# risc0/zeth

Measured on AMD Instinct MI355X. Metric: segments/sec, higher is better.
Workload: dtype u32

## Files before the change

### zeth_amd/csrc/common.h

```cpp
#pragma once
#include <hip/hip_runtime.h>

#include <atomic>
#include <cstdarg>
#include <cstdio>
#include <cstdlib>
#include <cstring>
#include <map>
#include <string>
#include <vector>

#include "../../include/zkhal.h"
#include "fp.h"
#include "noise.h"

namespace zkh {

inline const char* make_err(const char* fmt, ...) {
    char buf[512];
    va_list ap;
    va_start(ap, fmt);
    vsnprintf(buf, sizeof buf, fmt, ap);
    va_end(ap);
    return strdup(buf);
}
#define ZKH_HIP(expr)                                                                               \
    do {                                                                                            \
        hipError_t _e = (expr);                                                                     \
        if (_e != hipSuccess) return zkh::make_err("%s failed: %s (%s:%d)", #expr, hipGetErrorString(_e), __FILE__, __LINE__); \
    } while (0)
#define ZKH_TRY(expr)                    \
    do {                                 \
        const char* _err = (expr);       \
        if (_err) return _err;           \
    } while (0)
#define ZKH_REQUIRE(cond, ...)                         \
    do {                                               \
        if (!(cond)) return zkh::make_err(__VA_ARGS__); \
    } while (0)

constexpr int ZKH_P2_PTAB = 486;
constexpr int TW_BITS = 12;
constexpr int TW_SIZE = 1 << TW_BITS;
constexpr int TW_HI_BITS = 14;
constexpr int TW_HI_SIZE = 1 << TW_HI_BITS;
constexpr int MAX_LOG_N = TW_BITS + TW_HI_BITS;
constexpr int LDS_TW_LOG = 12;

struct DeviceTables {
    uint32_t* rc;
    uint32_t* diag;
    uint32_t* tw_fwd_lo; uint32_t* tw_fwd_hi;
    uint32_t* tw_rev_lo; uint32_t* tw_rev_hi;
    uint32_t* tile_fwd;  uint32_t* tile_rev;
    uint32_t* layer_fwd; uint32_t* layer_rev;
    uint32_t* layer_fwd_lazy;
    uint32_t* shift_lo;  uint32_t* shift_hi;
};

struct ProfAgg { uint64_t calls = 0; double ms = 0; double bytes = 0; };
struct ProfPending { std::string name; hipEvent_t a, b; double bytes; };

}

struct zkh_alloc_t {
    void* ptr;
    size_t bytes;
    std::atomic<int> refs;
    bool owned;
    zkh_ctx* ctx;
    zkh_alloc_t(void* p, size_t b, int r, bool o, zkh_ctx* c) : ptr(p), bytes(b), refs(r), owned(o), ctx(c) {}
};

struct zkh_buf {
    zkh_alloc_t* a;
    size_t off, len;
    std::atomic<int> refs;
    zkh_buf(zkh_alloc_t* al, size_t o, size_t l, int r) : a(al), off(o), len(l), refs(r) {}
    uint32_t* ptr() const { return (uint32_t*)a->ptr + off; }
};

struct zkh_ctx {
    int device;
    hipStream_t stream;
    zkh::DeviceTables tab;
    uint32_t rou_fwd[28], rou_rev[28];
    uint32_t h_rc[24 * 29], h_diag[zkh::ZKH_P2_PTAB];
    std::multimap<size_t, void*> pool;
    size_t pool_bytes = 0, live_bytes = 0, peak_bytes = 0;
    bool prof = false;
    std::vector<zkh::ProfPending> pending;
    std::map<std::string, zkh::ProfAgg> agg;
    std::vector<hipEvent_t> event_pool;
    uint32_t* pinned = nullptr;
    size_t pinned_words = 0;
    size_t stage_next = 0, stage_used = 0;
    uint32_t* d_fail = nullptr;
    uint32_t* h_fail = nullptr;
    bool fail_armed = false;
    std::map<void*, size_t> host_blocks;
    size_t h2d_bytes = 0;
};

namespace zkh {

const char* pool_alloc(zkh_ctx* c, size_t bytes, void** out);
void pool_free(zkh_ctx* c, void* p, size_t bytes);
const char* new_buf(zkh_ctx* c, size_t n_words, bool zero, zkh_buf** out);
void prof_begin(zkh_ctx* c, const char* name, double bytes);
void prof_end(zkh_ctx* c);
const char* ensure_pinned(zkh_ctx* c, size_t words);
const char* resolve_noise_key(const uint32_t* key_or_null, NoiseKey* out);

inline void bind_thread(const zkh_ctx* c) { (void)hipSetDevice(c->device); }
const char* ntt_device_init(zkh_ctx* c);

struct Tmp {
    zkh_buf* b = nullptr;
    Tmp() {}
    Tmp(const Tmp&) = delete;
    Tmp& operator=(const Tmp&) = delete;
    ~Tmp() { if (b) zkh_release(b); }
    zkh_buf** out() { if (b) { zkh_release(b); b = nullptr; } return &b; }
    operator zkh_buf*() const { return b; }
    zkh_buf* operator->() const { return b; }
    explicit operator bool() const { return b != nullptr; }
};

struct ProfScope {
    zkh_ctx* c;
    ProfScope(zkh_ctx* ctx, const char* name, double bytes) : c(ctx) { bind_thread(c); if (c->prof) prof_begin(c, name, bytes); }
    ~ProfScope() { if (c->prof) prof_end(c); }
};

inline const char* last_launch_error(const char* what) {
    hipError_t e = hipGetLastError();
    if (e != hipSuccess) return make_err("launch %s: %s", what, hipGetErrorString(e));
    return nullptr;
}

__device__ __forceinline__ uint32_t xcd_remap(uint32_t b, uint32_t nblocks) {
    const uint32_t xcd = b & 7u, q = nblocks >> 3, r = nblocks & 7u, idx = b >> 3;
    const uint32_t base = xcd < r ? xcd * (q + 1) : r * (q + 1) + (xcd - r) * q;
    return base + idx;
}

}
```

### zeth_amd/csrc/hash.hip

```cpp
#include "common.h"
#include "image_tree.h"
#include "poseidon2.h"
#include "poseidon2_wide.h"

using namespace zkh;

static_assert(zkh::ZKH_P2_PTAB == zkh::P2_TAB_WORDS, "common.h ZKH_P2_PTAB must equal poseidon2.h P2_TAB_WORDS");

namespace {

__global__ __launch_bounds__(256, 4) void k_hash_rows(uint32_t* __restrict__ out, const uint32_t* __restrict__ matrix,
                                                   size_t rows, uint32_t cols, const uint32_t* __restrict__ rc,
                                                   const uint32_t* __restrict__ diag) {
    const size_t r = (size_t)blockIdx.x * blockDim.x + threadIdx.x;
    if (r >= rows) return;
    uint32_t s[CELLS];
#pragma unroll
    for (int i = 0; i < CELLS; i++) s[i] = 0;
    const uint32_t* src = matrix + r;
    const uint32_t full = cols / RATE, tail = cols % RATE;
    const uint32_t blocks = full + (tail || cols == 0 ? 1u : 0u);
    for (uint32_t b = 0; b < blocks; b++) {
        const uint32_t* bsrc = src + (size_t)b * RATE * rows;
        if (b < full) {
#pragma unroll
            for (int i = 0; i < RATE; i++) s[i] = bsrc[(size_t)i * rows];
        } else {
#pragma unroll
            for (int i = 0; i < RATE; i++) s[i] = (uint32_t)i < tail ? bsrc[(size_t)i * rows] : 0u;
        }
        poseidon2_mix_sponge(s, rc, diag, b + 1 == blocks);
#pragma unroll
        for (int i = RATE; i < CELLS; i++) s[i] = p2_signed(s[i]);
    }
#pragma unroll
    for (int i = 0; i < OUT; i++) s[i] = canon((int32_t)s[RATE + i]);
    uint4* o = (uint4*)(out + r * 8);
    o[0] = make_uint4(s[0], s[1], s[2], s[3]);
    o[1] = make_uint4(s[4], s[5], s[6], s[7]);
}

__device__ __forceinline__ void fold_one(uint32_t* __restrict__ io, size_t input_size, size_t output_size, size_t i,
                                         const uint32_t* __restrict__ rc, const uint32_t* __restrict__ diag) {
    const uint4* src = (const uint4*)(io + (input_size + 2 * i) * 8);
    uint32_t s[CELLS];
    const uint4 a = src[0], b = src[1], c = src[2], d = src[3];
    s[0] = a.x; s[1] = a.y; s[2] = a.z; s[3] = a.w; s[4] = b.x; s[5] = b.y; s[6] = b.z; s[7] = b.w;
    s[8] = c.x; s[9] = c.y; s[10] = c.z; s[11] = c.w; s[12] = d.x; s[13] = d.y; s[14] = d.z; s[15] = d.w;
#pragma unroll
    for (int k = RATE; k < CELLS; k++) s[k] = 0;
    poseidon2_mix_raw<0, OUT, RATE>(s, rc, diag);
#pragma unroll
    for (int k = 0; k < OUT; k++) s[k] = p2_finish(s[k]);
    uint4* o = (uint4*)(io + (output_size + i) * 8);
    o[0] = make_uint4(s[0], s[1], s[2], s[3]);
    o[1] = make_uint4(s[4], s[5], s[6], s[7]);
}
__global__ __launch_bounds__(256, 4) void k_hash_fold(uint32_t* __restrict__ io, size_t input_size, size_t output_size,
                                                   const uint32_t* __restrict__ rc, const uint32_t* __restrict__ diag) {
    const size_t i = (size_t)blockIdx.x * blockDim.x + threadIdx.x;
    if (i >= output_size) return;
    fold_one(io, input_size, output_size, i, rc, diag);
}
__global__ __launch_bounds__(256, 4) void k_hash_fold_list(uint32_t* __restrict__ io, size_t width, const uint32_t* __restrict__ list,
                                                        const uint32_t* __restrict__ count, const uint32_t* __restrict__ rc,
                                                        const uint32_t* __restrict__ diag) {
    const uint32_t t = blockIdx.x * blockDim.x + threadIdx.x;
    if (t >= *count) return;
    fold_one(io, 2 * width, width, list[t], rc, diag);
}

__device__ __forceinline__ void wide_fold_one(uint32_t* __restrict__ io, size_t input_size, size_t output_size, uint32_t gid,
                                              const uint32_t* rcs, const uint32_t* __restrict__ pc) {
    const uint32_t j = gid & 7;
    size_t parent = gid >> 3;
    const bool live = parent < output_size;
    if (!live) parent = output_size - 1;
    uint32_t c[4] = {0, 0, 0, 0};
    if (j < 4) {
        const uint4 v = *(const uint4*)(io + (input_size + 2 * parent) * 8 + 4 * j);
        c[0] = v.x; c[1] = v.y; c[2] = v.z; c[3] = v.w;
    }
    wide_permute(c, j, rcs, pc);
    if (live && j < 2) *(uint4*)(io + (output_size + parent) * 8 + 4 * j) = make_uint4(c[0], c[1], c[2], c[3]);
}
constexpr int TAIL_LOG = 7;
__global__ __launch_bounds__(8 << TAIL_LOG) void k_hash_fold_subtree(uint32_t* __restrict__ io, size_t first_parents, uint32_t levels,
                                                                     const uint32_t* __restrict__ rc, const uint32_t* __restrict__ pc) {
    __shared__ __attribute__((aligned(16))) uint32_t rcs[ROUNDS_TOTAL * CELLS + 8];
    for (uint32_t w = threadIdx.x; w < ROUNDS_TOTAL * CELLS; w += blockDim.x) rcs[w] = rc[w];
    __syncthreads();
    for (uint32_t l = 0; l < levels; l++) {
        const size_t parents = first_parents >> l;
        const uint32_t local = (1u << TAIL_LOG) >> l;
        if ((threadIdx.x >> 6) * 8 < local) {
            const uint32_t grp = threadIdx.x >> 3;
            const uint32_t gid = grp < local ? (uint32_t)((blockIdx.x * local + grp) * 8 + (threadIdx.x & 7)) : 0xffffffffu;
            wide_fold_one(io, 2 * parents, parents, gid, rcs, pc);
        }
        __threadfence_block();
        __syncthreads();
    }
}
__global__ __launch_bounds__(8 << TAIL_LOG) void k_hash_fold_tail(uint32_t* __restrict__ io, size_t first_parents,
                                                                  const uint32_t* __restrict__ rc, const uint32_t* __restrict__ pc) {
    __shared__ __attribute__((aligned(16))) uint32_t rcs[ROUNDS_TOTAL * CELLS + 8];
    for (uint32_t w = threadIdx.x; w < ROUNDS_TOTAL * CELLS; w += blockDim.x) rcs[w] = rc[w];
    __syncthreads();
    for (size_t parents = first_parents; parents >= 1; parents >>= 1) {
        if ((threadIdx.x >> 6) * 8 < parents)
            wide_fold_one(io, 2 * parents, parents, threadIdx.x, rcs, pc);
        __threadfence_block();
        __syncthreads();
    }
}

__global__ __launch_bounds__(256) void k_poseidon2_mix(uint32_t* __restrict__ io, size_t count, const uint32_t* __restrict__ rc,
                                                       const uint32_t* __restrict__ diag) {
    const size_t i = (size_t)blockIdx.x * blockDim.x + threadIdx.x;
    if (i >= count) return;
    uint4* p = (uint4*)(io + i * CELLS);
    uint32_t s[CELLS];
#pragma unroll
    for (int q = 0; q < CELLS / 4; q++) { const uint4 v = p[q]; s[4 * q] = v.x; s[4 * q + 1] = v.y; s[4 * q + 2] = v.z; s[4 * q + 3] = v.w; }
    poseidon2_mix(s, rc, diag);
#pragma unroll
    for (int q = 0; q < CELLS / 4; q++) p[q] = make_uint4(s[4 * q], s[4 * q + 1], s[4 * q + 2], s[4 * q + 3]);
}

}

extern "C" const char* zkh_poseidon2_mix(zkh_ctx* c, zkh_buf* states, size_t count) {
    ZKH_REQUIRE(states && states->len == count * CELLS, "poseidon2_mix: buffer is not count x 24 words");
    if (!count) return nullptr;
    bind_thread(c);
    k_poseidon2_mix<<<(unsigned)((count + 255) / 256), 256, 0, c->stream>>>(states->ptr(), count, c->tab.rc, c->tab.diag);
    return last_launch_error("poseidon2_mix");
}
extern "C" const char* zkh_hash_rows(zkh_ctx* c, zkh_buf* out, const zkh_buf* matrix) {
    ZKH_REQUIRE(out->len % 8 == 0 && out->len, "hash_rows: output is not a digest array");
    const size_t rows = out->len / 8;
    ZKH_REQUIRE(matrix->len % rows == 0, "hash_rows: matrix size %zu not a multiple of rows %zu", matrix->len, rows);
    const size_t cols = matrix->len / rows;
    ProfScope prof(c, "hash_rows", 4.0 * matrix->len + 32.0 * rows);
    k_hash_rows<<<(unsigned)((rows + 255) / 256), 256, 0, c->stream>>>(out->ptr(), matrix->ptr(), rows, (uint32_t)cols,
                                                                      c->tab.rc, c->tab.diag);
    return last_launch_error("hash_rows");
}
extern "C" const char* zkh_hash_fold(zkh_ctx* c, zkh_buf* io, size_t input_size, size_t output_size) {
    ZKH_REQUIRE(io->len % 8 == 0, "hash_fold: not a digest array");
    ZKH_REQUIRE((input_size + 2 * output_size) * 8 <= io->len && output_size * 2 <= input_size, "hash_fold: ranges out of bounds");
    if (!output_size) return nullptr;
    ProfScope prof(c, "hash_fold", 96.0 * output_size);
    k_hash_fold<<<(unsigned)((output_size + 255) / 256), 256, 0, c->stream>>>(io->ptr(), input_size, output_size, c->tab.rc,
                                                                             c->tab.diag);
    return last_launch_error("hash_fold");
}
extern "C" const char* zkh_merkle_fold_all(zkh_ctx* c, zkh_buf* nodes, size_t rows) {
    ZKH_REQUIRE(nodes->len == rows * 16 && rows && (rows & (rows - 1)) == 0, "merkle_fold_all: nodes must hold 2*rows digests");
    return merkle_fold_from(c, nodes, rows);
}
extern "C" const char* zkh_merkle_build(zkh_ctx* c, zkh_buf* nodes, const zkh_buf* matrix, size_t rows) {
    ZKH_REQUIRE(nodes && matrix && nodes->len == rows * 16 && rows && (rows & (rows - 1)) == 0, "merkle_build: nodes must hold 2*rows digests");
    ZKH_REQUIRE(matrix->len % rows == 0, "merkle_build: matrix size %zu not a multiple of rows %zu", matrix->len, rows);
    zkh_buf* leaves = nullptr;
    ZKH_TRY(zkh_slice(nodes, rows * 8, rows * 8, &leaves));
    const char* err = zkh_hash_rows(c, leaves, matrix);
    zkh_release(leaves);
    ZKH_TRY(err);
    return merkle_fold_from(c, nodes, rows);
}
const char* zkh::merkle_fold_from(zkh_ctx* c, zkh_buf* nodes, size_t first_layer) {
    for (size_t layer = first_layer; layer >= 2; layer /= 2) {
        const size_t parents = layer / 2;
        if (parents > ((size_t)1 << WIDE_LOG)) {
            ZKH_TRY(zkh_hash_fold(c, nodes, layer, parents));
        } else if (parents > ((size_t)1 << TAIL_LOG)) {
            uint32_t levels = 0;
            while ((parents >> levels) > ((size_t)1 << TAIL_LOG)) levels++;
            ProfScope prof(c, "hash_fold_wide", 96.0 * (2 * parents - (parents >> (levels - 1))));
            k_hash_fold_subtree<<<(unsigned)(parents >> TAIL_LOG), 8 << TAIL_LOG, 0, c->stream>>>(nodes->ptr(), parents, levels, c->tab.rc,
                                                                                                   c->tab.diag);
            ZKH_TRY(last_launch_error("hash_fold_wide"));
            layer >>= (levels - 1);
        } else {
            ProfScope prof(c, "hash_fold_tail", 96.0 * (2 * parents - 1));
            k_hash_fold_tail<<<1, 8 << TAIL_LOG, 0, c->stream>>>(nodes->ptr(), parents, c->tab.rc, c->tab.diag);
            ZKH_TRY(last_launch_error("hash_fold_tail"));
            break;
        }
    }
    return nullptr;
}
const char* zkh::hash_fold_listed(zkh_ctx* c, zkh_buf* nodes, size_t width, const uint32_t* list, const uint32_t* count, uint32_t bound) {
    ZKH_REQUIRE(bound && bound <= width && 32 * width <= nodes->len, "hash_fold_listed: %u parents of %zu in %zu words", bound, width, nodes->len);
    ProfScope prof(c, "image_sparse", 100.0 * bound);
    k_hash_fold_list<<<(bound + 255) / 256, 256, 0, c->stream>>>(nodes->ptr(), width, list, count, c->tab.rc, c->tab.diag);
    return last_launch_error("image_sparse");
}
```

### zeth_amd/csrc/poseidon2.h

```cpp
#pragma once
#include "fp.h"

namespace zkh {

constexpr int CELLS = 24, RATE = 16, OUT = 8, HALF_FULL = 4, PARTIAL = 21, ROUNDS_TOTAL = 2 * HALF_FULL + PARTIAL;
constexpr int P2_TAB_SIGNED = 74, P2_TAB_FULL = P2_TAB_SIGNED + 3 * CELLS, P2_TAB_GROUP0 = P2_TAB_FULL + 2 * HALF_FULL * CELLS,
              P2_TAB_KAPPA = P2_TAB_GROUP0 + 3 * CELLS, P2_TAB_EXIT = P2_TAB_KAPPA + 4, P2_TAB_WORDS = P2_TAB_EXIT + 3 * CELLS;

ZKH_HD uint32_t sbox7_rc(uint32_t x, uint32_t rcs) {
    const int32_t sx = (int32_t)(x + rcs);
    const int32_t x2 = smont(sx, sx), x3 = smont(x2, sx), x4 = smont(x2, x2);
    return canon(smont(x3, x4));
}
ZKH_HD uint32_t dbl_mod(uint32_t x) {
#if defined(__HIP_DEVICE_COMPILE__)
    uint32_t d;
    asm("v_add_u32_e32 %0, %1, %1" : "=v"(d) : "v"(x));
    return reduce_once(d);
#else
    return reduce_once(x + x);
#endif
}
ZKH_HD void m4(uint32_t& x0, uint32_t& x1, uint32_t& x2, uint32_t& x3) {
    const uint32_t t0 = add_mod(x0, x1), t1 = add_mod(x2, x3);
    const uint32_t t2 = add_mod(dbl_mod(x1), t1), t3 = add_mod(dbl_mod(x3), t0);
    const uint32_t t4 = add_mod(dbl_mod(dbl_mod(t1)), t3), t5 = add_mod(dbl_mod(dbl_mod(t0)), t2);
    x0 = add_mod(t3, t5); x1 = t5; x2 = add_mod(t2, t4); x3 = t4;
}
ZKH_HD void m_ext(uint32_t (&s)[CELLS]) {
    uint32_t c0 = 0, c1 = 0, c2 = 0, c3 = 0;
#pragma unroll
    for (int i = 0; i < CELLS; i += 4) {
        m4(s[i], s[i + 1], s[i + 2], s[i + 3]);
        c0 = add_mod(c0, s[i]); c1 = add_mod(c1, s[i + 1]); c2 = add_mod(c2, s[i + 2]); c3 = add_mod(c3, s[i + 3]);
    }
#pragma unroll
    for (int i = 0; i < CELLS; i += 4) {
        s[i] = add_mod(s[i], c0); s[i + 1] = add_mod(s[i + 1], c1);
        s[i + 2] = add_mod(s[i + 2], c2); s[i + 3] = add_mod(s[i + 3], c3);
    }
}
constexpr uint32_t F64_OFF = 0x43380000u;
constexpr double F64_MAGIC = 6755399441055744.0;

ZKH_HD int64_t f64_bits(double d) {
#if defined(__HIP_DEVICE_COMPILE__)
    return __double_as_longlong(d);
#else
    int64_t b; __builtin_memcpy(&b, &d, 8); return b;
#endif
}
ZKH_HD double fmad(double a, double b, double c) {
#if defined(__HIP_DEVICE_COMPILE__)
    return __builtin_fma(a, b, c);
#else
    return a * b + c;
#endif
}
ZKH_HD void m4d(double& x0, double& x1, double& x2, double& x3) {
    const double t0 = x0 + x1, t1 = x2 + x3;
    const double t2 = fmad(x1, 2.0, t1), t3 = fmad(x3, 2.0, t0);
    const double t4 = fmad(t1, 4.0, t3), t5 = fmad(t0, 4.0, t2);
    x0 = t3 + t5; x1 = t5; x2 = t2 + t4; x3 = t4;
}
ZKH_HD uint32_t m_ext_f64_cell(double tm) {
    const int64_t t = f64_bits(tm);
    const int32_t m = (int32_t)((uint32_t)t * NEG_PINV);
    return (uint32_t)((uint64_t)mad_i64_k(m, (int32_t)P, t) >> 32);
}
template <int LIVE>
ZKH_HD void m_ext_f64_blocks(double (&d)[CELLS], double (&c)[4]) {
    static_assert(LIVE % 4 == 0 && LIVE > 0 && LIVE <= CELLS, "whole 4-cell blocks");
    c[0] = c[1] = c[2] = c[3] = F64_MAGIC;
#pragma unroll
    for (int i = 0; i < LIVE; i += 4) {
        m4d(d[i], d[i + 1], d[i + 2], d[i + 3]);
        c[0] += d[i]; c[1] += d[i + 1]; c[2] += d[i + 2]; c[3] += d[i + 3];
    }
}
template <int LIVE, int SRC_LO, int DST_LO, int N>
ZKH_HD void m_ext_f64_reduce(uint32_t (&s)[CELLS], const double (&d)[CELLS], const double (&c)[4]) {
    static_assert(SRC_LO % 4 == 0 && DST_LO % 4 == 0 && SRC_LO + N <= CELLS && DST_LO + N <= CELLS, "column-aligned cell range");
#pragma unroll
    for (int k = 0; k < N; k++) s[DST_LO + k] = m_ext_f64_cell(SRC_LO + k < LIVE ? d[SRC_LO + k] + c[k % 4] : c[k % 4]);
}
ZKH_HD void m_ext_f64(uint32_t (&s)[CELLS], double (&d)[CELLS]) {
    double c[4];
    m_ext_f64_blocks<CELLS>(d, c);
    m_ext_f64_reduce<CELLS, 0, 0, CELLS>(s, d, c);
}
ZKH_HD uint64_t fold64(uint64_t a, uint64_t t) {
#if defined(__HIP_DEVICE_COMPILE__)
    uint64_t d, carry;
    asm("v_mad_u64_u32 %0, %1, %2, %3, %4" : "=v"(d), "=s"(carry) : "v"((uint32_t)(a >> 32)), "s"(R1), "v"(t));
    asm("v_mad_u64_u32 %0, %1, %2, 1, %3" : "=v"(t), "=s"(carry) : "v"((uint32_t)a), "v"(d));
    return t;
#else
    return t + (a >> 32) * R1 + (uint32_t)a;
#endif
}
ZKH_HD int32_t sbox7_lazy(uint32_t v, uint32_t rcf) {
    const int32_t sx = (int32_t)(v + rcf);
    const int32_t x2 = smont(sx, sx), x3 = smont(x2, sx), x4 = smont(x2, x2);
    return smont(x3, x4);
}

inline uint32_t p2_mulm(uint32_t a, uint32_t b) { return (uint32_t)((uint64_t)a * b % P); }
inline uint32_t p2_powm(uint32_t a, uint64_t e) { uint32_t r = 1; while (e) { if (e & 1) r = p2_mulm(r, a); a = p2_mulm(a, a); e >>= 1; } return r; }
inline uint32_t p2_full_round_scale(uint32_t lambda) { return p2_mulm(p2_powm(lambda, 7), p2_powm(p2_powm(R1, P - 2), 7)); }
inline uint32_t p2_exit_scale() {
    uint64_t e = 0;
    for (uint64_t k = 1; k < 7 && !e; k++) if ((k * (P - 1) + 1) % 7 == 0) e = (k * (P - 1) + 1) / 7;
    uint32_t lambda = R1;
    for (int f = 0; f < HALF_FULL; f++) lambda = p2_mulm(p2_powm(lambda, e), R1);
    return lambda;
}
inline bool poseidon2_partial_table(uint32_t* t, const uint32_t* rc_canonical, const uint32_t* diag_canonical) {
    Fp c1 = Fp::zero();
    for (int i = 0; i < CELLS; i++) {
        const Fp d = fp_encode(diag_canonical[i]);
        t[i] = d.v; t[CELLS + i] = (d * d).v; t[2 * CELLS + i] = (d * d * d).v;
        if (i) c1 = c1 + d;
    }
    t[3 * CELLS] = c1.v; t[3 * CELLS + 1] = fp_encode(23).v;
    for (int i = 0; i < 3 * CELLS; i++) t[P2_TAB_SIGNED + i] = (uint32_t)center(t[i]);
    const uint32_t rinv = p2_powm(R1, P - 2);
    auto rneg = [&](uint64_t k) { return p2_powm(rinv, k); };
    const uint32_t sigma = p2_exit_scale();
    uint32_t lam[2 * HALF_FULL + 1] = {1u, rneg(7), rneg(56), rneg(399), sigma};
    for (int f = HALF_FULL; f < 2 * HALF_FULL; f++) lam[f + 1] = p2_full_round_scale(lam[f]);
    for (int f = 0; f < 2 * HALF_FULL; f++) {
        const int round = f < HALF_FULL ? f : HALF_FULL + PARTIAL + (f - HALF_FULL);
        for (int i = 0; i < CELLS; i++) {
            const uint32_t v = p2_mulm(lam[f], rc_canonical[round * CELLS + i] % P);
            t[P2_TAB_FULL + f * CELLS + i] = f == HALF_FULL ? v - P : (uint32_t)center(v) - F64_OFF;
        }
    }
    const uint32_t rho = p2_powm(R1, 2801);
    for (int i = 0; i < 3 * CELLS; i++) t[P2_TAB_GROUP0 + i] = (uint32_t)center(p2_mulm(t[i], rho));
    t[P2_TAB_KAPPA] = (uint32_t)center(p2_mulm(rho, R1));
    t[P2_TAB_KAPPA + 1] = p2_mulm(rho, R1);
    const uint32_t mu = p2_mulm(sigma, rinv);
    t[P2_TAB_KAPPA + 2] = sigma;
    t[P2_TAB_KAPPA + 3] = p2_mulm(t[0], mu);
    for (int i = 0; i < 3 * CELLS; i++) t[P2_TAB_EXIT + i] = (uint32_t)center(p2_mulm(t[i], mu));
    return lam[2 * HALF_FULL] == R1;
}
ZKH_HD uint32_t p2_signed(uint32_t v) { return v - F64_OFF; }
ZKH_HD uint32_t p2_finish(uint32_t v) { return canon((int32_t)p2_signed(v)); }
template <int KEEP_LO, int KEEP_N, int LIVE, bool SEL>
ZKH_HD void poseidon2_mix_core(uint32_t (&s)[CELLS], const uint32_t* __restrict__ rc, const uint32_t* __restrict__ diag, bool low) {
    static_assert(!SEL || KEEP_LO >= KEEP_N, "the two selectable ranges do not overlap");
    const uint32_t* __restrict__ rcf = diag + P2_TAB_FULL;
    double d[CELLS], c[4];
#pragma unroll
    for (int i = 0; i < LIVE; i++) d[i] = (double)(int32_t)s[i];
    m_ext_f64_blocks<LIVE>(d, c);
    m_ext_f64_reduce<LIVE, 0, 0, CELLS>(s, d, c);
#pragma unroll 1
    for (int r = 0; r < HALF_FULL; r++) {
#pragma unroll
        for (int i = 0; i < CELLS; i++) d[i] = (double)sbox7_lazy(s[i], rcf[r * CELLS + i]);
        m_ext_f64(s, d);
    }
    s[0] = canon(smont((int32_t)(s[0] - F64_OFF), (int32_t)diag[P2_TAB_KAPPA]));
#pragma unroll
    for (int i = 1; i < CELLS; i++) s[i] -= F64_OFF;
    int round = HALF_FULL;
    const uint32_t* __restrict__ pc = diag;
    const int32_t* __restrict__ pcs = (const int32_t*)(diag + P2_TAB_SIGNED);
    constexpr int64_t BIAS = (int64_t)((uint64_t)P << 32);
    constexpr int32_t R1S = (int32_t)R1;
#pragma unroll 1
    for (int grp = 0; grp < PARTIAL / 3; grp++, round += 3) {
        const bool last = grp == PARTIAL / 3 - 1;
        const int32_t* __restrict__ pcg = grp == 0 ? (const int32_t*)(diag + P2_TAB_GROUP0) : pcs;
        const int32_t* __restrict__ pcu = last ? (const int32_t*)(diag + P2_TAB_EXIT) : pcs;
        const int32_t* __restrict__ pcu3 = last ? pcu : pcg;
        int64_t ta = BIAS, tb = BIAS;
#pragma unroll
        for (int i = 1; i <= 12; i++) ta = mad_i64_k((int32_t)s[i], R1S, ta);
#pragma unroll
        for (int i = 13; i < CELLS; i++) tb = mad_i64_k((int32_t)s[i], R1S, tb);
        uint64_t a1[6], a2[6];
#pragma unroll
        for (int c = 0; c < 6; c++) {
            int64_t x1 = BIAS, x2 = BIAS;
#pragma unroll
            for (int i = 1 + 4 * c; i < 5 + 4 * c && i < CELLS; i++) {
                x1 = mad_i64_k((int32_t)s[i], pcg[i], x1);
                x2 = mad_i64_k((int32_t)s[i], pcg[CELLS + i], x2);
            }
            a1[c] = (uint64_t)x1; a2[c] = (uint64_t)x2;
        }
        const uint32_t d0 = pc[0], c1 = pc[3 * CELLS], m23 = pc[3 * CELLS + 1];
        const uint32_t z0 = sbox7_rc(s[0], rc[round * CELLS]);
        uint32_t S0;
        if (grp == 0)
            S0 = add_mod(z0, mul_mod(add_mod(mont_reduce_wide((uint64_t)ta), mont_reduce_wide((uint64_t)tb)), diag[P2_TAB_KAPPA + 1]));
        else
            S0 = mont_reduce(fold64((uint64_t)tb, fold64((uint64_t)ta, (uint64_t)z0 * R1)));
        const uint32_t s0a = mont_reduce_wide(((uint64_t)S0 << 32) + (uint64_t)d0 * z0);
        const uint32_t z1 = sbox7_rc(s0a, rc[(round + 1) * CELLS]);
        uint64_t t1 = (uint64_t)m23 * S0 + (uint64_t)z1 * R1;
#pragma unroll
        for (int c = 0; c < 6; c++) t1 = fold64(a1[c], t1);
        const uint32_t S1 = mont_reduce_wide(t1);
        const uint32_t s0b = mont_reduce_wide(((uint64_t)S1 << 32) + (uint64_t)d0 * z1);
        const uint32_t z2 = sbox7_rc(s0b, rc[(round + 2) * CELLS]);
        uint64_t t2 = (uint64_t)m23 * S1 + (uint64_t)c1 * S0 + (uint64_t)z2 * R1;
#pragma unroll
        for (int c = 0; c < 6; c++) t2 = fold64(a2[c], t2);
        uint32_t S2 = mont_reduce_wide(t2), d0u = d0;
        if (last) { S2 = mul_mod(S2, diag[P2_TAB_KAPPA + 2]); d0u = diag[P2_TAB_KAPPA + 3]; }
        s[0] = mont_reduce_wide(((uint64_t)S2 << 32) + (uint64_t)d0u * z2);
        const int32_t S0c = center(S0), S1c = center(S1);
        const int64_t acc0 = mad_i64_k(center(S2), R1S, 0);
#pragma unroll
        for (int i = 1; i < CELLS; i++)
            s[i] = (uint32_t)smont_reduce(mad_i64_k((int32_t)s[i], pcu3[2 * CELLS + i],
                                                    mad_i64_k(S0c, pcu[CELLS + i], mad_i64_k(S1c, pcu[i], acc0))));
    }
#pragma unroll
    for (int i = 1; i < CELLS; i++) s[i] = canon((int32_t)s[i]);
#pragma unroll 1
    for (int r = HALF_FULL; r < 2 * HALF_FULL - 1; r++) {
#pragma unroll
        for (int i = 0; i < CELLS; i++) d[i] = (double)sbox7_lazy(s[i], rcf[r * CELLS + i]);
        m_ext_f64(s, d);
    }
#pragma unroll
    for (int i = 0; i < CELLS; i++) d[i] = (double)sbox7_lazy(s[i], rcf[(2 * HALF_FULL - 1) * CELLS + i]);
    m_ext_f64_blocks<CELLS>(d, c);
    if (SEL && low) m_ext_f64_reduce<CELLS, 0, KEEP_LO, KEEP_N>(s, d, c);
    else            m_ext_f64_reduce<CELLS, KEEP_LO, KEEP_LO, KEEP_N>(s, d, c);
}
template <int KEEP_LO = 0, int KEEP_N = CELLS, int LIVE = CELLS>
ZKH_HD void poseidon2_mix_raw(uint32_t (&s)[CELLS], const uint32_t* __restrict__ rc, const uint32_t* __restrict__ diag) {
    poseidon2_mix_core<KEEP_LO, KEEP_N, LIVE, false>(s, rc, diag, false);
}
ZKH_HD void poseidon2_mix_sponge(uint32_t (&s)[CELLS], const uint32_t* __restrict__ rc, const uint32_t* __restrict__ diag, bool last_block) {
    poseidon2_mix_core<RATE, OUT, CELLS, true>(s, rc, diag, last_block);
}
ZKH_HD void poseidon2_mix(uint32_t (&s)[CELLS], const uint32_t* __restrict__ rc, const uint32_t* __restrict__ diag) {
    poseidon2_mix_raw(s, rc, diag);
#pragma unroll
    for (int i = 0; i < CELLS; i++) s[i] = p2_finish(s[i]);
}

}
```

Baseline: 44.70.

## Carry sponge capacity as unreduced doubles between Poseidon2 row-hash blocks

The row-hash sponge now keeps the 8 capacity cells as unreduced f64 linear-layer outputs between blocks. This skips the final modular reduction and the re-entry canonicalisation on interior blocks, and it uses precomputed alternate exit scaling tables so the Montgomery factor comes out as one. The last external layer also computes only the kept 4-cell blocks instead of reducing all 24 cells. The cost is extra table entries, a more complex template path, and more live double registers per thread, which could lower occupancy.

New measurement: 44.47. Within noise of the previous version (-0.5%).

```diff
diff --git a/zeth_amd/csrc/common.h b/zeth_amd/csrc/common.h
--- a/zeth_amd/csrc/common.h
+++ b/zeth_amd/csrc/common.h
@@ -39,7 +39,7 @@
         if (!(cond)) return zkh::make_err(__VA_ARGS__); \
     } while (0)
 
-constexpr int ZKH_P2_PTAB = 486;
+constexpr int ZKH_P2_PTAB = 656;
 constexpr int TW_BITS = 12;
 constexpr int TW_SIZE = 1 << TW_BITS;
 constexpr int TW_HI_BITS = 14;
diff --git a/zeth_amd/csrc/hash.hip b/zeth_amd/csrc/hash.hip
--- a/zeth_amd/csrc/hash.hip
+++ b/zeth_amd/csrc/hash.hip
@@ -14,14 +14,15 @@
                                                    const uint32_t* __restrict__ diag) {
     const size_t r = (size_t)blockIdx.x * blockDim.x + threadIdx.x;
     if (r >= rows) return;
-    uint32_t s[CELLS];
-#pragma unroll
-    for (int i = 0; i < CELLS; i++) s[i] = 0;
+    double cap[OUT];
+#pragma unroll
+    for (int i = 0; i < OUT; i++) cap[i] = 0.0;
     const uint32_t* src = matrix + r;
     const uint32_t full = cols / RATE, tail = cols % RATE;
     const uint32_t blocks = full + (tail || cols == 0 ? 1u : 0u);
     for (uint32_t b = 0; b < blocks; b++) {
         const uint32_t* bsrc = src + (size_t)b * RATE * rows;
+        uint32_t s[CELLS];
         if (b < full) {
 #pragma unroll
             for (int i = 0; i < RATE; i++) s[i] = bsrc[(size_t)i * rows];
@@ -29,15 +30,15 @@
 #pragma unroll
             for (int i = 0; i < RATE; i++) s[i] = (uint32_t)i < tail ? bsrc[(size_t)i * rows] : 0u;
         }
-        poseidon2_mix_sponge(s, rc, diag, b + 1 == blocks);
-#pragma unroll
-        for (int i = RATE; i < CELLS; i++) s[i] = p2_signed(s[i]);
-    }
-#pragma unroll
-    for (int i = 0; i < OUT; i++) s[i] = canon((int32_t)s[RATE + i]);
-    uint4* o = (uint4*)(out + r * 8);
-    o[0] = make_uint4(s[0], s[1], s[2], s[3]);
-    o[1] = make_uint4(s[4], s[5], s[6], s[7]);
+        poseidon2_mix_carry(s, cap, rc, diag, b == 0, b + 1 == blocks);
+        if (b + 1 == blocks) {
+#pragma unroll
+            for (int i = 0; i < OUT; i++) s[i] = p2_finish(s[RATE + i]);
+            uint4* o = (uint4*)(out + r * 8);
+            o[0] = make_uint4(s[0], s[1], s[2], s[3]);
+            o[1] = make_uint4(s[4], s[5], s[6], s[7]);
+        }
+    }
 }
 
 __device__ __forceinline__ void fold_one(uint32_t* __restrict__ io, size_t input_size, size_t output_size, size_t i,
diff --git a/zeth_amd/csrc/poseidon2.h b/zeth_amd/csrc/poseidon2.h
--- a/zeth_amd/csrc/poseidon2.h
+++ b/zeth_amd/csrc/poseidon2.h
@@ -5,7 +5,9 @@
 
 constexpr int CELLS = 24, RATE = 16, OUT = 8, HALF_FULL = 4, PARTIAL = 21, ROUNDS_TOTAL = 2 * HALF_FULL + PARTIAL;
 constexpr int P2_TAB_SIGNED = 74, P2_TAB_FULL = P2_TAB_SIGNED + 3 * CELLS, P2_TAB_GROUP0 = P2_TAB_FULL + 2 * HALF_FULL * CELLS,
-              P2_TAB_KAPPA = P2_TAB_GROUP0 + 3 * CELLS, P2_TAB_EXIT = P2_TAB_KAPPA + 4, P2_TAB_WORDS = P2_TAB_EXIT + 3 * CELLS;
+              P2_TAB_KAPPA = P2_TAB_GROUP0 + 3 * CELLS, P2_TAB_EXIT = P2_TAB_KAPPA + 4, P2_TAB_FULL_C = P2_TAB_EXIT + 3 * CELLS,
+              P2_TAB_KAPPA_C = P2_TAB_FULL_C + HALF_FULL * CELLS, P2_TAB_EXIT_C = P2_TAB_KAPPA_C + 2,
+              P2_TAB_WORDS = P2_TAB_EXIT_C + 3 * CELLS;
 
 ZKH_HD uint32_t sbox7_rc(uint32_t x, uint32_t rcs) {
     const int32_t sx = (int32_t)(x + rcs);
@@ -88,6 +90,20 @@
     double c[4];
     m_ext_f64_blocks<CELLS>(d, c);
     m_ext_f64_reduce<CELLS, 0, 0, CELLS>(s, d, c);
+}
+ZKH_HD void m_ext_f64_blocksum(double (&x)[4], const double (&d)[CELLS]) {
+#pragma unroll
+    for (int k = 0; k < 4; k++) x[k] = ((d[k] + d[4 + k]) + (d[8 + k] + d[12 + k])) + (d[16 + k] + d[20 + k]);
+}
+template <int LO, int NB>
+ZKH_HD void m_ext_f64_kept(double (&t)[4 * NB], const double (&d)[CELLS], const double (&x)[4]) {
+    static_assert(LO % 4 == 0 && NB > 0 && LO + 4 * NB <= CELLS, "whole 4-cell blocks");
+#pragma unroll
+    for (int b = 0; b < NB; b++) {
+#pragma unroll
+        for (int k = 0; k < 4; k++) t[4 * b + k] = d[LO + 4 * b + k] + x[k];
+        m4d(t[4 * b], t[4 * b + 1], t[4 * b + 2], t[4 * b + 3]);
+    }
 }
 ZKH_HD uint64_t fold64(uint64_t a, uint64_t t) {
 #if defined(__HIP_DEVICE_COMPILE__)
@@ -108,10 +124,10 @@
 inline uint32_t p2_mulm(uint32_t a, uint32_t b) { return (uint32_t)((uint64_t)a * b % P); }
 inline uint32_t p2_powm(uint32_t a, uint64_t e) { uint32_t r = 1; while (e) { if (e & 1) r = p2_mulm(r, a); a = p2_mulm(a, a); e >>= 1; } return r; }
 inline uint32_t p2_full_round_scale(uint32_t lambda) { return p2_mulm(p2_powm(lambda, 7), p2_powm(p2_powm(R1, P - 2), 7)); }
-inline uint32_t p2_exit_scale() {
+inline uint32_t p2_exit_scale(uint32_t out = R1) {
     uint64_t e = 0;
     for (uint64_t k = 1; k < 7 && !e; k++) if ((k * (P - 1) + 1) % 7 == 0) e = (k * (P - 1) + 1) / 7;
-    uint32_t lambda = R1;
+    uint32_t lambda = out;
     for (int f = 0; f < HALF_FULL; f++) lambda = p2_mulm(p2_powm(lambda, e), R1);
     return lambda;
 }
@@ -126,37 +142,63 @@
     for (int i = 0; i < 3 * CELLS; i++) t[P2_TAB_SIGNED + i] = (uint32_t)center(t[i]);
     const uint32_t rinv = p2_powm(R1, P - 2);
     auto rneg = [&](uint64_t k) { return p2_powm(rinv, k); };
-    const uint32_t sigma = p2_exit_scale();
-    uint32_t lam[2 * HALF_FULL + 1] = {1u, rneg(7), rneg(56), rneg(399), sigma};
-    for (int f = HALF_FULL; f < 2 * HALF_FULL; f++) lam[f + 1] = p2_full_round_scale(lam[f]);
-    for (int f = 0; f < 2 * HALF_FULL; f++) {
+    auto full_row = [&](uint32_t* row, int f, uint32_t lambda) {
         const int round = f < HALF_FULL ? f : HALF_FULL + PARTIAL + (f - HALF_FULL);
         for (int i = 0; i < CELLS; i++) {
-            const uint32_t v = p2_mulm(lam[f], rc_canonical[round * CELLS + i] % P);
-            t[P2_TAB_FULL + f * CELLS + i] = f == HALF_FULL ? v - P : (uint32_t)center(v) - F64_OFF;
-        }
-    }
+            const uint32_t v = p2_mulm(lambda, rc_canonical[round * CELLS + i] % P);
+            row[i] = f == HALF_FULL ? v - P : (uint32_t)center(v) - F64_OFF;
+        }
+    };
+    const uint32_t lam[HALF_FULL] = {1u, rneg(7), rneg(56), rneg(399)};
+    for (int f = 0; f < HALF_FULL; f++) full_row(t + P2_TAB_FULL + f * CELLS, f, lam[f]);
     const uint32_t rho = p2_powm(R1, 2801);
     for (int i = 0; i < 3 * CELLS; i++) t[P2_TAB_GROUP0 + i] = (uint32_t)center(p2_mulm(t[i], rho));
     t[P2_TAB_KAPPA] = (uint32_t)center(p2_mulm(rho, R1));
     t[P2_TAB_KAPPA + 1] = p2_mulm(rho, R1);
-    const uint32_t mu = p2_mulm(sigma, rinv);
-    t[P2_TAB_KAPPA + 2] = sigma;
-    t[P2_TAB_KAPPA + 3] = p2_mulm(t[0], mu);
-    for (int i = 0; i < 3 * CELLS; i++) t[P2_TAB_EXIT + i] = (uint32_t)center(p2_mulm(t[i], mu));
-    return lam[2 * HALF_FULL] == R1;
+    auto exit_rows = [&](uint32_t sigma, uint32_t* full, uint32_t* kappa, uint32_t* rows) {
+        uint32_t lambda = sigma;
+        for (int f = HALF_FULL; f < 2 * HALF_FULL; f++) {
+            full_row(full + (f - HALF_FULL) * CELLS, f, lambda);
+            lambda = p2_full_round_scale(lambda);
+        }
+        const uint32_t mu = p2_mulm(sigma, rinv);
+        kappa[0] = sigma;
+        kappa[1] = p2_mulm(t[0], mu);
+        for (int i = 0; i < 3 * CELLS; i++) rows[i] = (uint32_t)center(p2_mulm(t[i], mu));
+        return lambda;
+    };
+    const uint32_t out = exit_rows(p2_exit_scale(), t + P2_TAB_FULL + HALF_FULL * CELLS, t + P2_TAB_KAPPA + 2, t + P2_TAB_EXIT);
+    const uint32_t out_c = exit_rows(p2_exit_scale(1u), t + P2_TAB_FULL_C, t + P2_TAB_KAPPA_C, t + P2_TAB_EXIT_C);
+    return out == R1 && out_c == 1u;
 }
 ZKH_HD uint32_t p2_signed(uint32_t v) { return v - F64_OFF; }
 ZKH_HD uint32_t p2_finish(uint32_t v) { return canon((int32_t)p2_signed(v)); }
-template <int KEEP_LO, int KEEP_N, int LIVE, bool SEL>
-ZKH_HD void poseidon2_mix_core(uint32_t (&s)[CELLS], const uint32_t* __restrict__ rc, const uint32_t* __restrict__ diag, bool low) {
+template <int KEEP_LO, int KEEP_N, int LIVE, bool SEL, bool CARRY = false>
+ZKH_HD void poseidon2_mix_core(uint32_t (&s)[CELLS], const uint32_t* __restrict__ rc, const uint32_t* __restrict__ diag, bool low,
+                               double (&cap)[OUT], bool first) {
+    static_assert(KEEP_LO % 4 == 0, "the kept cells start at a block");
     static_assert(!SEL || KEEP_LO >= KEEP_N, "the two selectable ranges do not overlap");
+    static_assert(!CARRY || (SEL && KEEP_LO == RATE && KEEP_N == OUT && LIVE == RATE), "the carried capacity is cells 16..23");
     const uint32_t* __restrict__ rcf = diag + P2_TAB_FULL;
+    const bool interior = CARRY && !low;
     double d[CELLS], c[4];
 #pragma unroll
     for (int i = 0; i < LIVE; i++) d[i] = (double)(int32_t)s[i];
     m_ext_f64_blocks<LIVE>(d, c);
-    m_ext_f64_reduce<LIVE, 0, 0, CELLS>(s, d, c);
+    if (CARRY) {
+#pragma unroll
+        for (int i = 0; i < OUT; i++) d[RATE + i] = cap[i];
+        if (!first) {
+#pragma unroll
+            for (int i = RATE; i < CELLS; i += 4) {
+                m4d(d[i], d[i + 1], d[i + 2], d[i + 3]);
+                c[0] += d[i]; c[1] += d[i + 1]; c[2] += d[i + 2]; c[3] += d[i + 3];
+            }
+        }
+        m_ext_f64_reduce<CELLS, 0, 0, CELLS>(s, d, c);
+    } else {
+        m_ext_f64_reduce<LIVE, 0, 0, CELLS>(s, d, c);
+    }
 #pragma unroll 1
     for (int r = 0; r < HALF_FULL; r++) {
 #pragma unroll
@@ -175,7 +217,7 @@
     for (int grp = 0; grp < PARTIAL / 3; grp++, round += 3) {
         const bool last = grp == PARTIAL / 3 - 1;
         const int32_t* __restrict__ pcg = grp == 0 ? (const int32_t*)(diag + P2_TAB_GROUP0) : pcs;
-        const int32_t* __restrict__ pcu = last ? (const int32_t*)(diag + P2_TAB_EXIT) : pcs;
+        const int32_t* __restrict__ pcu = last ? (const int32_t*)(diag + (interior ? P2_TAB_EXIT_C : P2_TAB_EXIT)) : pcs;
         const int32_t* __restrict__ pcu3 = last ? pcu : pcg;
         int64_t ta = BIAS, tb = BIAS;
 #pragma unroll
@@ -212,7 +254,10 @@
 #pragma unroll
         for (int c = 0; c < 6; c++) t2 = fold64(a2[c], t2);
         uint32_t S2 = mont_reduce_wide(t2), d0u = d0;
-        if (last) { S2 = mul_mod(S2, diag[P2_TAB_KAPPA + 2]); d0u = diag[P2_TAB_KAPPA + 3]; }
+        if (last) {
+            const uint32_t* __restrict__ kap = diag + (interior ? P2_TAB_KAPPA_C : P2_TAB_KAPPA + 2);
+            S2 = mul_mod(S2, kap[0]); d0u = kap[1];
+        }
         s[0] = mont_reduce_wide(((uint64_t)S2 << 32) + (uint64_t)d0u * z2);
         const int32_t S0c = center(S0), S1c = center(S1);
         const int64_t acc0 = mad_i64_k(center(S2), R1S, 0);
@@ -223,24 +268,43 @@
     }
 #pragma unroll
     for (int i = 1; i < CELLS; i++) s[i] = canon((int32_t)s[i]);
+    const uint32_t* __restrict__ rcs = interior ? diag + (P2_TAB_FULL_C - HALF_FULL * CELLS) : rcf;
 #pragma unroll 1
     for (int r = HALF_FULL; r < 2 * HALF_FULL - 1; r++) {
 #pragma unroll
-        for (int i = 0; i < CELLS; i++) d[i] = (double)sbox7_lazy(s[i], rcf[r * CELLS + i]);
+        for (int i = 0; i < CELLS; i++) d[i] = (double)sbox7_lazy(s[i], rcs[r * CELLS + i]);
         m_ext_f64(s, d);
     }
 #pragma unroll
-    for (int i = 0; i < CELLS; i++) d[i] = (double)sbox7_lazy(s[i], rcf[(2 * HALF_FULL - 1) * CELLS + i]);
-    m_ext_f64_blocks<CELLS>(d, c);
-    if (SEL && low) m_ext_f64_reduce<CELLS, 0, KEEP_LO, KEEP_N>(s, d, c);
-    else            m_ext_f64_reduce<CELLS, KEEP_LO, KEEP_LO, KEEP_N>(s, d, c);
+    for (int i = 0; i < CELLS; i++) d[i] = (double)sbox7_lazy(s[i], rcs[(2 * HALF_FULL - 1) * CELLS + i]);
+    constexpr int NB = (KEEP_N + 3) / 4;
+    double x[4], t[4 * NB];
+    m_ext_f64_blocksum(x, d);
+    if (interior) {
+        m_ext_f64_kept<RATE, OUT / 4>(cap, d, x);
+    } else {
+        if (SEL && low) m_ext_f64_kept<0, NB>(t, d, x);
+        else            m_ext_f64_kept<KEEP_LO, NB>(t, d, x);
+#pragma unroll
+        for (int k = 0; k < KEEP_N; k++) s[KEEP_LO + k] = m_ext_f64_cell(t[k] + F64_MAGIC);
+        if (CARRY) {
+#pragma unroll
+            for (int k = 0; k < OUT; k++) cap[k] = 0.0;
+        }
+    }
 }
 template <int KEEP_LO = 0, int KEEP_N = CELLS, int LIVE = CELLS>
 ZKH_HD void poseidon2_mix_raw(uint32_t (&s)[CELLS], const uint32_t* __restrict__ rc, const uint32_t* __restrict__ diag) {
-    poseidon2_mix_core<KEEP_LO, KEEP_N, LIVE, false>(s, rc, diag, false);
+    double unused[OUT];
+    poseidon2_mix_core<KEEP_LO, KEEP_N, LIVE, false>(s, rc, diag, false, unused, false);
 }
 ZKH_HD void poseidon2_mix_sponge(uint32_t (&s)[CELLS], const uint32_t* __restrict__ rc, const uint32_t* __restrict__ diag, bool last_block) {
-    poseidon2_mix_core<RATE, OUT, CELLS, true>(s, rc, diag, last_block);
+    double unused[OUT];
+    poseidon2_mix_core<RATE, OUT, CELLS, true>(s, rc, diag, last_block, unused, false);
+}
+ZKH_HD void poseidon2_mix_carry(uint32_t (&s)[CELLS], double (&cap)[OUT], const uint32_t* __restrict__ rc, const uint32_t* __restrict__ diag,
+                                bool first_block, bool last_block) {
+    poseidon2_mix_core<RATE, OUT, RATE, true, true>(s, rc, diag, last_block, cap, first_block);
 }
 ZKH_HD void poseidon2_mix(uint32_t (&s)[CELLS], const uint32_t* __restrict__ rc, const uint32_t* __restrict__ diag) {
     poseidon2_mix_raw(s, rc, diag);
```
